# ZhengyiLuo/PHC

Measured on AMD Instinct MI355X. Metric: env-steps/sec at 4096 humanoid envs per GPU (VecEnv.step incl. resets), higher is better.
Workload: dtype f32

## Files before the change

### phc_amd/csrc/phc_im.h

```cpp
#pragma once
#include "phc_task.h"

namespace phc {

#if defined(PHC_SIM_PROFILE) && defined(__HIPCC__)
static __device__ unsigned long long g_phc_ptl[32];
static __device__ long long g_phc_ptl_env = -1;
#if defined(__HIP_DEVICE_COMPILE__)
#define PHC_PTL(i, ENV, LANE) if ((long long)(ENV) == g_phc_ptl_env) { __builtin_amdgcn_sched_barrier(0); __builtin_amdgcn_s_waitcnt(0); \
        const unsigned long long t_ = __builtin_readcyclecounter(); if ((LANE) == 0) g_phc_ptl[i] = t_; __builtin_amdgcn_sched_barrier(0); }
#else
#define PHC_PTL(i, ENV, LANE)
#endif
#else
#define PHC_PTL(i, ENV, LANE)
#endif

PHC_HD int64_t motion_id_of(const phc_im_buffers_t& buf, int64_t env) { return buf.sampled_motion_ids ? buf.sampled_motion_ids[env] : env; }

PHC_HD int phc_atomic_inc(int32_t* p) {
#if defined(__HIP_DEVICE_COMPILE__)
    return atomicAdd(p, 1);
#else
    int v;
// ... 200 lines not shown
    const Q4 hroot = obs_root_rot(prm, root.rot);
    Q4 hinv = calc_heading_quat_inv(hroot), h = calc_heading_quat(hroot);
    float* obs = buf.obs_buf + env * (int64_t)(prm.num_self_obs + prm.num_task_obs);
    if (prm.self_obs_v == 2 && buf.body_state_hist) self_obs_v2_lane(prm, buf.body_state_hist, nb, env, j, body, root, hinv, obs, true, false);
    else self_obs_lane(prm, nb, j, body, root, hinv, obs, (sim.force_sensor && prm.self_obs_v == 3) ? sim.force_sensor + env * (int64_t)(prm.num_force_sensors * 6) : nullptr, env);
    PHC_PTL(4, env, j)
    {
        float* amp = buf.amp_obs_out + env * amp_env_stride(prm, buf);
        amp_obs_from_sim_lane(prm, sim, nb, nd, env, j, root, hinv, model.ints + 4 + 3 * PHC_MAX_BODIES, amp);
    }
    PHC_PTL(5, env, j)
    BodyState r0 = ref_body_blend(q0, fr0.blend), r1 = ref_body_blend(q1, fr1.blend);
    r0.pos += c.goff; r1.pos += c.goff;
    rp = reward_partial(prm, env, nb, j, body, r0);
    if (c.cycled) {
        BodyState rr = ref_body(lib, frame_ref(lib, mid, c.t_rew), j);
        rr.pos += c.goff_rew;
        RewardPartial q = reward_partial(prm, env, nb, j, body, rr);
        rp.pos = q.pos; rp.rot = q.rot; rp.vel = q.vel; rp.angvel = q.angvel;
        if (j == 0) rp.root_dist = norm(body.pos - rr.pos);
    } else if (j == 0) {
        rp.root_dist = norm(body.pos - r0.pos);
    }
    if (prm.track_body_reward && prm.track_slot[j] < 0) rp.pos = rp.rot = rp.vel = rp.angvel = 0.f;
    if (occluded(buf, prm, env, prm.track_slot[j])) { rp.dist = 0.f; rp.fallen = 0; }
    if (prm.power_reward && j >= 1) {
        int ds = model.ints[4 + 3 * PHC_MAX_BODIES + j];
        const float* d = sim.dof_state + (env * nd + ds) * 2;
        const float* f = sim.dof_force + env * nd + ds;
        rp.power = fabsf(f[0] * d[1]);
        if (prm.dofs_per_joint != 1) rp.power += fabsf(f[1] * d[3]) + fabsf(f[2] * d[5]);
    }
    PHC_PTL(6, env, j)
    int slot = prm.track_slot[j];
    if (slot >= 0) {
        BodyState rt = r1;
        if (prm.zero_out_far && !(prm.obs_v >= 1 && prm.obs_v <= 3)) {
            BodyState rroot = (j == 0) ? r1 : ref_body(lib, fr1, 0);
            if (j != 0) rroot.pos += c.goff;
            const float dist = zero_out_far_ref(prm, slot, body, root, rroot, &rt);
            if (j == 0 && buf.point_goal) buf.point_goal[env] = dist;
        }
        occlude_ref(buf, prm, env, slot, body, &rt);
        V3 jd = v3(0.f, 0.f, 0.f), jv, rjd = jd, rjv;
        if (prm.obs_v == 2 && j >= 1) {
            ld_joint_state(sim, nd, env, model.ints[4 + 3 * PHC_MAX_BODIES + j], prm.dofs_per_joint, &jd, &jv);
            ref_joint(lib, fr1, j, &rjd, &rjv);
        }
        task_obs_lane(prm, slot, body, root, rt, hinv, h, obs + prm.num_self_obs, &jd, &rjd);
    }
    PHC_PTL(7, env, j)
    if (buf.ref_body_pos) st3(buf.ref_body_pos + (env * nb + j) * 3, r1.pos);
    if (buf.ref_body_rot) st4(buf.ref_body_rot + (env * nb + j) * 4, r1.rot);
    if (buf.ref_body_vel) st3(buf.ref_body_vel + (env * nb + j) * 3, r1.vel);
    if (want_dof)
        st_joint(buf.ref_dof_pos + env * nd + model.ints[4 + 3 * PHC_MAX_BODIES + j], prm.dofs_per_joint, ref_joint_pos_blend(lib, qj, fr1.blend));
    PHC_PTL(8, env, j)
    if (prm.num_traj_samples > 1)
        task_obs_future_lane(lib, prm, mid, c.progress + 1, c.start, c.start_off, c.goff, prm.track_slot[j], j, load_body(sim.rigid_body_state, env, nb, j),
                             load_body(sim.rigid_body_state, env, nb, 0), buf.obs_buf + env * (int64_t)(prm.num_self_obs + prm.num_task_obs) + prm.num_self_obs);
    return rp;
}

PHC_HD void im_post_finalize(const phc_motion_lib_t& lib, const phc_im_params_t& prm, const phc_im_buffers_t& buf, int nb,
                             int64_t env, const ImStepCtx& c, int64_t progress, float s_pos, float s_rot, float s_vel, float s_angvel,
                             float s_power, float s_dist, float root_dist, float prev_point_goal, int any_fallen, int n_reset_bodies) {
    float J = (float)nb, JE = (float)(nb + prm.num_ext_bodies);
    if (prm.track_body_reward) J = JE = (float)prm.num_track_bodies;
    float r_pos = expf(-prm.k_pos * (s_pos / JE));
    float r_rot = expf(-prm.k_rot * (s_rot / JE));
    float r_vel = expf(-prm.k_vel * (s_vel / J));
    float r_ang = expf(-prm.k_ang_vel * (s_angvel / J));
    float rew = prm.w_pos * r_pos + prm.w_rot * r_rot + prm.w_vel * r_vel + prm.w_ang_vel * r_ang;
    const int nraw = prm.power_reward ? 5 : 4;
    float* raw = buf.reward_raw + env * nraw;
    if (prm.zero_out_far) {
        const float pg = fminf(prev_point_goal - root_dist, 1.0f / 3.0f) * 9.0f;
        const bool far = root_dist > 0.25f;
        raw[0] = pg + (far ? 0.f : r_pos * 0.5f);
        raw[1] = far ? 0.f : r_rot * 0.5f; raw[2] = far ? 0.f : r_vel * 0.5f; raw[3] = far ? 0.f : r_ang * 0.5f;
        rew = pg + (far ? 0.f : rew * 0.5f);
    } else {
        raw[0] = r_pos; raw[1] = r_rot; raw[2] = r_vel; raw[3] = r_ang;
    }
    if (prm.power_reward) {
        float pr = -prm.power_coefficient * s_power;
        if (progress <= 3) pr = 0.f;
        rew += pr;
        raw[4] = pr;
    }
    buf.rew_buf[env] = rew;
    int fallen = any_fallen;
    if (prm.use_mean_termination) {
        float mean = s_dist / (float)n_reset_bodies;
        fallen = mean > prm.termination_distances[prm.first_reset_body] ? 1 : 0;
    }
    int64_t terminated = 0;
    if (prm.enable_early_termination) {
        if (!(progress > 1)) fallen = 0;
        if (prm.disable_collision_check) fallen = 0;
        terminated = fallen ? 1 : 0;
    }
    int64_t reset = c.pass_time ? 1 : terminated;
    if (!c.pass_time && c.cycle_cnt > 0) { reset = 0; terminated = 0; }
    if (c.recovery_cnt > 0) { reset = 0; terminated = 0; }
    buf.terminate_buf[env] = terminated;
    buf.reset_buf[env] = reset;
    if (reset && buf.reset_list) {
        const int sub = (int)((env >> 3) & (PHC_RESET_SUBLISTS - 1));
        const int i = phc_atomic_inc(buf.reset_count + (buf.reset_slot * PHC_RESET_SUBLISTS + sub) * PHC_RESET_COUNT_STRIDE);
        buf.reset_list[sub * buf.reset_sublist_cap + i] = (int32_t)env;
    }
    buf.progress_buf[env] = c.progress;
    if (buf.cycle_counter) buf.cycle_counter[env] = c.cycle_cnt;
    if (buf.recovery_counter) buf.recovery_counter[env] = c.recovery_cnt;
    if (c.cycled) {
        buf.motion_start_times[env] = c.start;
        buf.motion_start_times_offset[env] = c.start_off;
        st3(buf.global_offset + env * 3, c.goff);
    }
}

PHC_HD void im_reset_lane(const phc_model_t& model, const phc_motion_lib_t& lib, const phc_im_params_t& prm,
                          const phc_sim_state_t& sim, const phc_im_buffers_t& buf, int64_t env, int j, float t, bool clear_reset_flag,
                          int parts = 3) {
    const int nb = model.num_bodies, nd = model.num_dof;
    const int64_t mid = motion_id_of(buf, env);
    const bool p_state = (parts & 1) != 0, p_task = (parts & 2) != 0;
    if (j < nb) {
        const FrameRef fr = frame_ref(lib, mid, t);
        BodyState rs = ref_body(lib, fr, j);
        BodyState root = (j == 0) ? rs : ref_body(lib, fr, 0);
        if (p_state) {
        store_body(sim.rigid_body_state, env, nb, j, rs);
        if (sim.contact_force) st3(sim.contact_force + (env * nb + j) * 3, v3(0.f, 0.f, 0.f));
        if (j == 0) {
            float* r = sim.root_states + env * 13;
            st3(r, rs.pos); st4(r + 3, rs.rot); st3(r + 7, rs.vel); st3(r + 10, rs.angvel);
        } else {
            V3 dp, dv;
            ref_joint(lib, fr, j, &dp, &dv);
            const int ds = model.ints[4 + 3 * PHC_MAX_BODIES + j];
            float* d = sim.dof_state + (env * nd + ds) * 2;
            d[0] = dp.x; d[1] = dv.x;
            if (prm.dofs_per_joint != 1) { d[2] = dp.y; d[3] = dv.y; d[4] = dp.z; d[5] = dv.z; }
            st_joint(sim.pd_target + env * nd + ds, prm.dofs_per_joint, dp);
            if (sim.dof_force) st_joint(sim.dof_force + env * nd + ds, prm.dofs_per_joint, v3(0.f, 0.f, 0.f));
        }
        }
        const Q4 hroot = obs_root_rot(prm, root.rot);
        Q4 hinv = calc_heading_quat_inv(hroot), h = calc_heading_quat(hroot);
        float* obs = buf.obs_buf + env * (int64_t)(prm.num_self_obs + prm.num_task_obs);
        if (p_state) {
        if (prm.self_obs_v == 2 && buf.body_state_hist) self_obs_v2_lane(prm, buf.body_state_hist, nb, env, j, rs, root, hinv, obs, false, true);
        else self_obs_lane(prm, nb, j, rs, root, hinv, obs, (sim.force_sensor && prm.self_obs_v == 3) ? sim.force_sensor + env * (int64_t)(prm.num_force_sensors * 6) : nullptr, env);
        }
        if (p_task) {
        const float t1 = motion_time(1, prm.dt, t, 0.f);
        const FrameRef fr1 = frame_ref(lib, mid, t1);
        BodyState r1 = ref_body(lib, fr1, j);
        V3 goff = v3(0.f, 0.f, 0.f);
        if (buf.offset_rand && prm.zero_out_far && prm.zero_out_far_train)
            disk_offset(buf.offset_rand[env * 2], buf.offset_rand[env * 2 + 1], &goff.x, &goff.y);
        r1.pos += goff;
        int slot = prm.track_slot[j];
        if (slot >= 0) {
            BodyState rt = r1;
            if (prm.zero_out_far && !(prm.obs_v >= 1 && prm.obs_v <= 3)) {
                BodyState rroot = (j == 0) ? r1 : ref_body(lib, fr1, 0);
                if (j != 0) rroot.pos += goff;
                const float dist = zero_out_far_ref(prm, slot, rs, root, rroot, &rt);
                if (j == 0 && buf.point_goal) buf.point_goal[env] = dist;
            }
            occlude_ref(buf, prm, env, slot, rs, &rt);
            V3 jd = v3(0.f, 0.f, 0.f), jv, rjd = jd, rjv;
            if (prm.obs_v == 2 && j >= 1) { ref_joint(lib, fr, j, &jd, &jv); ref_joint(lib, fr1, j, &rjd, &rjv); }
            task_obs_lane(prm, slot, rs, root, rt, hinv, h, obs + prm.num_self_obs, &jd, &rjd);
        }
        if (buf.ref_body_pos) st3(buf.ref_body_pos + (env * nb + j) * 3, r1.pos);
        if (buf.ref_body_rot) st4(buf.ref_body_rot + (env * nb + j) * 4, r1.rot);
        if (buf.ref_body_vel) st3(buf.ref_body_vel + (env * nb + j) * 3, r1.vel);
        if (buf.ref_dof_pos && j >= 1) {
            V3 dp, dv;
            ref_joint(lib, fr1, j, &dp, &dv);
            st_joint(buf.ref_dof_pos + env * nd + model.ints[4 + 3 * PHC_MAX_BODIES + j], prm.dofs_per_joint, dp);
        }
        if (prm.num_traj_samples > 1) {
            const FrameRef frt = frame_ref(lib, mid, t);
            V3 go = v3(0.f, 0.f, 0.f);
            if (buf.offset_rand && prm.zero_out_far && prm.zero_out_far_train) disk_offset(buf.offset_rand[env * 2], buf.offset_rand[env * 2 + 1], &go.x, &go.y);
            task_obs_future_lane(lib, prm, mid, 1, t, 0.f, go, prm.track_slot[j], j, ref_body(lib, frt, j), ref_body(lib, frt, 0),
                                 buf.obs_buf + env * (int64_t)(prm.num_self_obs + prm.num_task_obs) + prm.num_self_obs);
        }
        }
    }
    if (j == 0 && p_state) {
        buf.motion_start_times[env] = t;
        buf.motion_start_times_offset[env] = 0.f;
        V3 goff = v3(0.f, 0.f, 0.f);
        const bool far_start = buf.offset_rand && prm.zero_out_far && prm.zero_out_far_train;
        if (far_start) disk_offset(buf.offset_rand[env * 2], buf.offset_rand[env * 2 + 1], &goff.x, &goff.y);
        st3(buf.global_offset + env * 3, goff);
        buf.progress_buf[env] = 0; buf.terminate_buf[env] = 0;
        if (clear_reset_flag) buf.reset_buf[env] = 0;
        if (buf.cycle_counter) buf.cycle_counter[env] = far_start ? prm.zero_out_far_steps : 0;
        if (buf.recovery_counter) buf.recovery_counter[env] = 0;
    }
}

PHC_HD void im_reset_from_state_lane(const phc_model_t& model, const phc_motion_lib_t& lib, const phc_im_params_t& prm,
                                     const phc_sim_state_t& sim, const phc_im_buffers_t& buf, int64_t env, int j, int fill_history) {
    const int nb = model.num_bodies, nd = model.num_dof;
    const int64_t mid = motion_id_of(buf, env);
    const int S = prm.num_amp_obs_steps, A = prm.num_amp_obs_per_step;
    if (j < nb) {
        BodyState body = load_body(sim.rigid_body_state, env, nb, j);
        BodyState root = load_body(sim.rigid_body_state, env, nb, 0);
        if (sim.contact_force) st3(sim.contact_force + (env * nb + j) * 3, v3(0.f, 0.f, 0.f));
        if (j >= 1) {
            const int ds = model.ints[4 + 3 * PHC_MAX_BODIES + j];
            V3 dp, dv;
            ld_joint_state(sim, nd, env, ds, prm.dofs_per_joint, &dp, &dv);
            st_joint(sim.pd_target + env * nd + ds, prm.dofs_per_joint, dp);
        }
        const V3 goff = ld3(buf.global_offset + env * 3);
        const float t1 = motion_time(1, prm.dt, buf.motion_start_times[env], buf.motion_start_times_offset[env]);
        const FrameRef fr1 = frame_ref(lib, mid, t1);
        BodyState r1 = ref_body(lib, fr1, j);
        r1.pos += goff;
        const Q4 hroot = obs_root_rot(prm, root.rot);
    Q4 hinv = calc_heading_quat_inv(hroot), h = calc_heading_quat(hroot);
        float* obs = buf.obs_buf + env * (int64_t)(prm.num_self_obs + prm.num_task_obs);
        if (prm.self_obs_v == 2 && buf.body_state_hist) self_obs_v2_lane(prm, buf.body_state_hist, nb, env, j, body, root, hinv, obs, false, true);
        else self_obs_lane(prm, nb, j, body, root, hinv, obs, (sim.force_sensor && prm.self_obs_v == 3) ? sim.force_sensor + env * (int64_t)(prm.num_force_sensors * 6) : nullptr, env);
        int slot = prm.track_slot[j];
        if (slot >= 0) {
            BodyState rt = r1;
            if (prm.zero_out_far && !(prm.obs_v >= 1 && prm.obs_v <= 3)) {
                BodyState rroot = (j == 0) ? r1 : ref_body(lib, fr1, 0);
                if (j != 0) rroot.pos += goff;
                const float dist = zero_out_far_ref(prm, slot, body, root, rroot, &rt);
                if (j == 0 && buf.point_goal) buf.point_goal[env] = dist;
            }
            occlude_ref(buf, prm, env, slot, body, &rt);
            V3 jd = v3(0.f, 0.f, 0.f), jv, rjd = jd, rjv;
            if (prm.obs_v == 2 && j >= 1) {
                ld_joint_state(sim, nd, env, model.ints[4 + 3 * PHC_MAX_BODIES + j], prm.dofs_per_joint, &jd, &jv);
                ref_joint(lib, fr1, j, &rjd, &rjv);
            }
            task_obs_lane(prm, slot, body, root, rt, hinv, h, obs + prm.num_self_obs, &jd, &rjd);
        }
        if (buf.ref_body_pos) st3(buf.ref_body_pos + (env * nb + j) * 3, r1.pos);
        if (buf.ref_body_rot) st4(buf.ref_body_rot + (env * nb + j) * 4, r1.rot);
        if (buf.ref_body_vel) st3(buf.ref_body_vel + (env * nb + j) * 3, r1.vel);
        if (buf.ref_dof_pos && j >= 1) {
            V3 dp, dv;
            ref_joint(lib, fr1, j, &dp, &dv);
            st_joint(buf.ref_dof_pos + env * nd + model.ints[4 + 3 * PHC_MAX_BODIES + j], prm.dofs_per_joint, dp);
        }
        float* amp = buf.amp_obs_out + env * amp_env_stride(prm, buf);
        const int nfill = fill_history ? S : 1;
        for (int k = 0; k < nfill; ++k)
            amp_obs_from_sim_lane(prm, sim, nb, nd, env, j, root, hinv, model.ints + 4 + 3 * PHC_MAX_BODIES, amp + k * A);
        if (prm.num_traj_samples > 1)
            task_obs_future_lane(lib, prm, mid, 1, buf.motion_start_times[env], buf.motion_start_times_offset[env], ld3(buf.global_offset + env * 3),
                                 prm.track_slot[j], j, load_body(sim.rigid_body_state, env, nb, j), load_body(sim.rigid_body_state, env, nb, 0),
                                 buf.obs_buf + env * (int64_t)(prm.num_self_obs + prm.num_task_obs) + prm.num_self_obs);
    }
    if (j == 0) {
        buf.progress_buf[env] = 0; buf.terminate_buf[env] = 0; buf.reset_buf[env] = 0;
    }
}

PHC_HD void im_reset_amp_lane(const phc_motion_lib_t& lib, const phc_im_params_t& prm, const phc_im_buffers_t& buf, int nb,
                              int64_t env, int j, float t, int k) {
    const int A = prm.num_amp_obs_per_step;
    float* amp = buf.amp_obs_out + env * amp_env_stride(prm, buf);
    amp_obs_from_ref_lane(lib, prm, nb, j, motion_id_of(buf, env), history_time(t, prm.dt, k), amp + k * A);
}
#define PHC_AMP_TABLE_BLEND_TOL 1e-4f
PHC_HD void amp_obs_from_table_lane(const phc_motion_lib_t& lib, const phc_im_params_t& prm, int nb, int j, int nl, int64_t mid, float t, float* a) {
    const int A = prm.num_amp_obs_per_step, E = prm.num_amp_obs_extra, W = A - E;
    const FrameRef fr = frame_ref(lib, mid, t);
    const float b = fr.blend;
    if (j < nb && E > 0 && prm.amp_obs_extra) obs_extra_lane(prm.amp_obs_extra + mid * E, E, j, nb, a + W);
    if (!(b <= PHC_AMP_TABLE_BLEND_TOL)) {
        amp_obs_from_frames_lane(lib, prm, nb, j, fr, a);
        return;
    }
    const float* r0 = prm.amp_ref_table + fr.f0 * (int64_t)W;
    const float* r1 = prm.amp_ref_table + fr.f1 * (int64_t)W;
    const float s0 = 1.0f - b;
    for (int c0 = j; c0 < W; c0 += 8 * nl) {
        float u[8], v[8];
        for (int i = 0; i < 8; ++i) { const int c = c0 + i * nl; if (c < W) { u[i] = r0[c]; v[i] = r1[c]; } }
        for (int i = 0; i < 8; ++i) { const int c = c0 + i * nl; if (c < W) a[c] = s0 * u[i] + b * v[i]; }
    }
}
PHC_HD void im_reset_amp_table_lane(const phc_motion_lib_t& lib, const phc_im_params_t& prm, const phc_im_buffers_t& buf, int nb,
                                    int64_t env, int j, int nl, float t, int k) {
    amp_obs_from_table_lane(lib, prm, nb, j, nl, motion_id_of(buf, env), history_time(t, prm.dt, k),
                            buf.amp_obs_out + env * amp_env_stride(prm, buf) + k * prm.num_amp_obs_per_step);
}

}
```

### phc_amd/csrc/phc_kernels.hip

```cpp
#include <hip/hip_runtime.h>
#include <stdlib.h>
#include "phc_aba.h"
#include "phc_im.h"

using namespace phc;

template <int CTRL>
__device__ __forceinline__ int dpp_i(int v) { return __builtin_amdgcn_update_dpp(0, v, CTRL, 0xf, 0xf, true); }
template <int G>
__device__ __forceinline__ float group_sum(float v) {
    v += __int_as_float(dpp_i<0xB1>(__float_as_int(v)));
    v += __int_as_float(dpp_i<0x4E>(__float_as_int(v)));
    v += __int_as_float(dpp_i<0x141>(__float_as_int(v)));
    v += __int_as_float(dpp_i<0x140>(__float_as_int(v)));
#pragma unroll
    for (int m = 16; m < G; m <<= 1) v += __shfl_xor(v, m, G);
    return v;
}
template <int G>
__device__ __forceinline__ int group_or(int v) {
    v |= dpp_i<0xB1>(v); v |= dpp_i<0x4E>(v); v |= dpp_i<0x141>(v); v |= dpp_i<0x140>(v);
#pragma unroll
    for (int m = 16; m < G; m <<= 1) v |= __shfl_xor(v, m, G);
    return v;
}

template <int DPJ>
__device__ __forceinline__ void pin_family(phc_motion_lib_t& lib, phc_im_params_t& prm) {
    lib.dofs_per_joint = DPJ; prm.dofs_per_joint = DPJ;
    if (DPJ == 3) { lib.num_ext_bodies = 0; prm.num_ext_bodies = 0; }
}

template <int DPJ, int G>
__global__ __launch_bounds__(256) void k_im_post_physics(phc_model_t model, phc_motion_lib_t lib, phc_im_params_t prm,
                                                        phc_sim_state_t sim, phc_im_buffers_t buf, int n_reset_bodies) {
    pin_family<DPJ>(lib, prm);
    const int lane = threadIdx.x & (G - 1);
    const int64_t env = ((int64_t)blockIdx.x * blockDim.x + threadIdx.x) / G;
    if (env >= sim.num_envs) return;
    PHC_PTL(0, env, lane)
    if (blockIdx.x == 0 && threadIdx.x == 0 && buf.reset_rng_counter) *buf.reset_rng_counter += 1;
    const int64_t progress = buf.progress_buf[env] + 1;
    const FrameTab tab = frame_tab(lib, motion_id_of(buf, env));
    const int jb = lane < model.num_bodies ? lane : 0;
    const BodyState body = load_body(sim.rigid_body_state, env, model.num_bodies, jb);
    const BodyState root = load_body(sim.rigid_body_state, env, model.num_bodies, 0);
    const ImStepCtx c = im_post_prologue(lib, prm, sim, buf, env, progress);
    const float prev_goal = (prm.zero_out_far && buf.point_goal) ? buf.point_goal[env] : 0.f;
    PHC_PTL(1, env, lane)
    RewardPartial rp = im_post_lane(model, lib, prm, sim, buf, env, lane, c, tab, body, root);
    PHC_PTL(9, env, lane)
    amp_shift_lane(prm, buf, env, lane, G);
    float s_pos = group_sum<G>(rp.pos), s_rot = group_sum<G>(rp.rot), s_vel = group_sum<G>(rp.vel), s_ang = group_sum<G>(rp.angvel);
    float s_pow = group_sum<G>(rp.power), s_dist = group_sum<G>(rp.dist);
    int fallen = group_or<G>(rp.fallen);
    PHC_PTL(10, env, lane)
    if (lane == 0)
        im_post_finalize(lib, prm, buf, model.num_bodies, env, c, progress, s_pos, s_rot, s_vel, s_ang, s_pow, s_dist, rp.root_dist,
                         prev_goal, fallen, n_reset_bodies);
    PHC_PTL(11, env, lane)
}
#ifdef PHC_SIM_PROFILE
extern "C" int32_t phc_debug_post_timeline(unsigned long long* out32, long long env) {
    if (out32 && hipMemcpyFromSymbol(out32, HIP_SYMBOL(phc::g_phc_ptl), sizeof(unsigned long long) * 32) != hipSuccess) return -1;
    unsigned long long z[32] = {0};
    if (hipMemcpyToSymbol(HIP_SYMBOL(phc::g_phc_ptl), z, sizeof(z)) != hipSuccess) return -1;
    return hipMemcpyToSymbol(HIP_SYMBOL(phc::g_phc_ptl_env), &env, sizeof(env)) == hipSuccess ? 0 : -1;
}
#endif

template <int DPJ, int G>
__global__ __launch_bounds__(256) void k_amp_ref_table(phc_model_t model, phc_motion_lib_t lib, phc_im_params_t prm, int64_t num_frames,
                                                       const int64_t* __restrict__ next_frame, float* __restrict__ table) {
    pin_family<DPJ>(lib, prm);
    const int lane = threadIdx.x & (G - 1);
    const int64_t f = ((int64_t)blockIdx.x * blockDim.x + threadIdx.x) / G;
    if (f >= num_frames) return;
    FrameRef fr;
    fr.f0 = f; fr.f1 = next_frame[f]; fr.idx0 = fr.idx1 = 0; fr.blend = 0.f;
    amp_obs_from_frames_lane(lib, prm, model.num_bodies, lane, fr, table + f * (int64_t)(prm.num_amp_obs_per_step - prm.num_amp_obs_extra));
}

template <int G>
__global__ __launch_bounds__(256) void k_im_reset_from_state(phc_model_t model, phc_motion_lib_t lib, phc_im_params_t prm, phc_sim_state_t sim,
                                                            phc_im_buffers_t buf, int num_reset, const int64_t* __restrict__ env_ids,
                                                            int fill_history) {
    const int lane = threadIdx.x & (G - 1);
    const int64_t r = ((int64_t)blockIdx.x * blockDim.x + threadIdx.x) / G;
    if (r >= num_reset) return;
    im_reset_from_state_lane(model, lib, prm, sim, buf, env_ids[r], lane, fill_history);
}

__device__ __forceinline__ float hash_u01(uint64_t key, uint32_t env) {
    uint32_t x = env * 0x9E3779B1u ^ (uint32_t)key;
    x ^= x >> 16; x *= 0x85EBCA6Bu; x ^= x >> 13; x *= 0xC2B2AE35u; x ^= x >> 16;
    x += (uint32_t)(key >> 32);
    x ^= x >> 15; x *= 0x2C1B3C6Du; x ^= x >> 12; x *= 0x297A2D39u; x ^= x >> 15;
    return (float)(x >> 8) * (1.0f / 16777216.0f);
}
__host__ __device__ static inline uint64_t splitmix64(uint64_t z) {
    z += 0x9E3779B97F4A7C15ull;
    z = (z ^ (z >> 30)) * 0xBF58476D1CE4E5B9ull;
    z = (z ^ (z >> 27)) * 0x94D049BB133111EBull;
    return z ^ (z >> 31);
}

#ifdef PHC_SIM_PROFILE
__device__ unsigned long long g_phc_rtl[64];
__device__ int g_phc_rtl_group = -1;
extern "C" int32_t phc_debug_reset_timeline(unsigned long long* out64, int32_t group) {
    if (out64 && hipMemcpyFromSymbol(out64, HIP_SYMBOL(g_phc_rtl), sizeof(g_phc_rtl)) != hipSuccess) return -1;
    unsigned long long z[64] = {0};
    if (hipMemcpyToSymbol(HIP_SYMBOL(g_phc_rtl), z, sizeof(z)) != hipSuccess) return -1;
    return hipMemcpyToSymbol(HIP_SYMBOL(g_phc_rtl_group), &group, sizeof(group)) == hipSuccess ? 0 : -1;
}
#define PHC_RTL(i) if (rtl_on) { __builtin_amdgcn_sched_barrier(0); __builtin_amdgcn_s_waitcnt(0); const unsigned long long t_ = __builtin_readcyclecounter(); \
        if (lane == 0) g_phc_rtl[i] = t_; __builtin_amdgcn_sched_barrier(0); }
#else
#define PHC_RTL(i)
#endif

template <int DPJ, bool RNG, int G>
__global__ __launch_bounds__(256) void k_im_reset(phc_model_t model, phc_motion_lib_t lib, phc_im_params_t prm, phc_sim_state_t sim,
                                                 phc_im_buffers_t buf, int num_reset, const int64_t* __restrict__ env_ids,
                                                 const float* __restrict__ phase, int start_at_zero, uint64_t rng_key) {
    pin_family<DPJ>(lib, prm);
    const int lane = threadIdx.x & (G - 1);
    const int64_t r = ((int64_t)blockIdx.x * blockDim.x + threadIdx.x) / G;
    const int k = (int)blockIdx.y;
#ifdef PHC_SIM_PROFILE
    const bool rtl_on = (int)(r * 16 + k) == g_phc_rtl_group;
#endif
    PHC_RTL(0)
    int64_t env;
    if (RNG && buf.reset_list) {
        const int cap = buf.reset_sublist_cap, r32 = (int)r;
        const int sub = r32 & (PHC_RESET_SUBLISTS - 1), i = r32 >> 4;
        if (r32 < PHC_RESET_SUBLISTS && k == 0 && lane == 0)
            buf.reset_count[(((buf.reset_slot + 1) % 3) * PHC_RESET_SUBLISTS + r32) * PHC_RESET_COUNT_STRIDE] = 0;
        if (i >= cap || i >= buf.reset_count[(buf.reset_slot * PHC_RESET_SUBLISTS + sub) * PHC_RESET_COUNT_STRIDE]) return;
        env = buf.reset_list[sub * cap + i];
    } else {
        if (r >= num_reset) return;
        env = env_ids ? env_ids[r] : r;
        if (!env_ids && buf.reset_buf[env] == 0) return;
    }
    PHC_RTL(1)
    const int64_t mid = motion_id_of(buf, env);
    const uint64_t key = (RNG && buf.reset_rng_counter) ? splitmix64(rng_key ^ (*buf.reset_rng_counter * 0x9E6C63D0876A9A47ull)) : rng_key;
    const float t = start_at_zero ? 0.f : sample_time_interval(lib, mid, RNG ? hash_u01(key, (uint32_t)env) : phase[r]);
    PHC_RTL(2)
    if (k < 2) im_reset_lane(model, lib, prm, sim, buf, env, lane, t, env_ids != nullptr, 1 << k);
    PHC_RTL(3)
    if (k >= 2) {
        if (prm.amp_ref_table != nullptr) im_reset_amp_table_lane(lib, prm, buf, model.num_bodies, env, lane, G, t, k - 2);
        else im_reset_amp_lane(lib, prm, buf, model.num_bodies, env, lane, t, k - 2);
    }
    PHC_RTL(4)
}

template <int G>
__global__ __launch_bounds__(256) void k_amp_obs_demo(phc_model_t model, phc_motion_lib_t lib, phc_im_params_t prm, int n,
                                                     const int64_t* __restrict__ motion_ids, const float* __restrict__ times0,
                                                     float* __restrict__ out) {
    const int lane = threadIdx.x & (G - 1);
    const int64_t i = ((int64_t)blockIdx.x * blockDim.x + threadIdx.x) / G;
    const int k = (int)blockIdx.y;
    const int S = prm.num_amp_obs_steps, A = prm.num_amp_obs_per_step;
    if (i >= n) return;
    if (prm.amp_ref_table != nullptr) amp_obs_from_table_lane(lib, prm, model.num_bodies, lane, G, motion_ids[i], history_time(times0[i], prm.dt, k), out + (i * S + k) * A);
    else amp_obs_from_ref_lane(lib, prm, model.num_bodies, lane, motion_ids[i], history_time(times0[i], prm.dt, k), out + (i * S + k) * A);
}

template <int G>
__global__ __launch_bounds__(256) void k_motion_state(phc_motion_lib_t lib, int n, const int64_t* __restrict__ ids,
                                                     const float* __restrict__ times, const float* __restrict__ offset,
                                                     float* rg_pos, float* rb_rot, float* body_vel, float* body_ang_vel,
                                                     float* dof_pos, float* dof_vel, int64_t* idx0, int64_t* idx1, float* blend,
                                                     float* rg_pos_ext, float* rb_rot_ext) {
    const int lane = threadIdx.x & (G - 1);
    const int64_t i = ((int64_t)blockIdx.x * blockDim.x + threadIdx.x) / G;
    if (i >= n) return;
    const int nb = lib.num_bodies;
    const FrameRef fr = frame_ref(lib, ids[i], times[i]);
    if (lane == 0) {
        if (idx0) idx0[i] = fr.idx0;
        if (idx1) idx1[i] = fr.idx1;
        if (blend) blend[i] = fr.blend;
    }
    if (lane >= nb) {
        const int e = lane - nb, ne = lib.num_ext_bodies;
        if (e < ne && (rg_pos_ext || rb_rot_ext)) {
            V3 p; Q4 q;
            ref_body_ext(lib, fr, e, &p, &q);
            if (offset) p += ld3(offset + i * 3);
            if (rg_pos_ext) st3(rg_pos_ext + (i * ne + e) * 3, p);
            if (rb_rot_ext) st4(rb_rot_ext + (i * ne + e) * 4, q);
        }
        return;
    }
    BodyState s = ref_body(lib, fr, lane);
    if (offset) s.pos += ld3(offset + i * 3);
    if (rg_pos) st3(rg_pos + (i * nb + lane) * 3, s.pos);
    if (rb_rot) st4(rb_rot + (i * nb + lane) * 4, s.rot);
    if (body_vel) st3(body_vel + (i * nb + lane) * 3, s.vel);
    if (body_ang_vel) st3(body_ang_vel + (i * nb + lane) * 3, s.angvel);
    if (lane >= 1 && (dof_pos || dof_vel)) {
        V3 dp, dv;
        ref_joint(lib, fr, lane, &dp, &dv);
        const int dpj = lib.dofs_per_joint == 1 ? 1 : 3;
        if (dof_pos) st_joint(dof_pos + (i * (nb - 1) + (lane - 1)) * dpj, dpj, dp);
        if (dof_vel) st_joint(dof_vel + (i * (nb - 1) + (lane - 1)) * dpj, dpj, dv);
    }
}

__global__ void k_sample_time_interval(phc_motion_lib_t lib, int n, const int64_t* __restrict__ ids,
                                       const float* __restrict__ phase, float* __restrict__ out) {
    const int i = blockIdx.x * blockDim.x + threadIdx.x;
    if (i < n) out[i] = sample_time_interval(lib, ids[i], phase[i]);
}

__global__ void k_gae(int T, int n, const float* __restrict__ fdones, const float* __restrict__ values,
                      const float* __restrict__ rewards, const float* __restrict__ next_values, float gamma, float tau,
                      float* __restrict__ advs) {
    const int i = blockIdx.x * blockDim.x + threadIdx.x;
    if (i >= n) return;
    float last = 0.f;
    for (int t = T - 1; t >= 0; --t) {
        const int64_t k = (int64_t)t * n + i;
        const float not_done = 1.0f - fdones[k];
        const float delta = rewards[k] + gamma * next_values[k] - values[k];
        last = delta + gamma * tau * not_done * last;
        advs[k] = last;
    }
}

__device__ __forceinline__ Q4 pl_quat_mul_norm(Q4 a, Q4 b) {
    Q4 q = quat_mul16(a, b);
    if (q.w < 0.f) q = q4(-q.x, -q.y, -q.z, -q.w);
    float n = fmaxf(sqrtf(q.x * q.x + q.y * q.y + q.z * q.z + q.w * q.w), 1e-9f);
    return q4(q.x / n, q.y / n, q.z / n, q.w / n);
}
__global__ void k_fk(phc_model_t model, int64_t T, const float* __restrict__ local_rot, const float* __restrict__ root_trans,
                     float* __restrict__ grot, float* __restrict__ gpos) {
    const int64_t f = (int64_t)blockIdx.x * blockDim.x + threadIdx.x;
    if (f >= T) return;
    const int nb = model.num_bodies;
    for (int j = 0; j < nb; ++j) {
        const int p = model_tab(model, 0, j);
        Q4 lq = ld4(local_rot + (f * nb + j) * 4);
        if (p < 0) {
            st4(grot + (f * nb + j) * 4, lq);
            st3(gpos + (f * nb + j) * 3, ld3(root_trans + f * 3));
        } else {
            Q4 pq = ld4(grot + (f * nb + p) * 4);
            const float* mb = model_body(model, j);
            V3 off = quat_rotate(pq, v3(mb[0], mb[1], mb[2]));
            st4(grot + (f * nb + j) * 4, pl_quat_mul_norm(pq, lq));
            st3(gpos + (f * nb + j) * 3, off + ld3(gpos + (f * nb + p) * 3));
        }
    }
}

static inline int32_t launch_status() {
    hipError_t e = hipGetLastError();
    return e == hipSuccess ? 0 : (int32_t)e;
}
static inline int env_blocks(int64_t groups, int lanes) { return (int)((groups * lanes + 255) / 256); }
static inline int group_lanes(int num_bodies, int num_ext) { return num_bodies + num_ext > 32 ? 64 : 32; }

extern "C" {

int32_t phc_abi_version(void) { return PHC_ABI_VERSION; }

int32_t phc_motion_state(const phc_motion_lib_t* lib, int32_t n, const int64_t* motion_ids, const float* motion_times,
                         const float* offset, float* rg_pos, float* rb_rot, float* body_vel, float* body_ang_vel,
                         float* dof_pos, float* dof_vel, int64_t* frame_idx0, int64_t* frame_idx1, float* blend, float* rg_pos_ext,
                         float* rb_rot_ext, void* stream) {
    if (!lib || n < 0 || lib->num_bodies + lib->num_ext_bodies > PHC_MAX_BODIES) return PHC_EINVAL;
    if (n == 0) return 0;
    if (group_lanes(lib->num_bodies, lib->num_ext_bodies) == 64)
        hipLaunchKernelGGL(k_motion_state<64>, dim3(env_blocks(n, 64)), dim3(256), 0, (hipStream_t)stream, *lib, n, motion_ids, motion_times, offset,
                           rg_pos, rb_rot, body_vel, body_ang_vel, dof_pos, dof_vel, frame_idx0, frame_idx1, blend, rg_pos_ext, rb_rot_ext);
    else
        hipLaunchKernelGGL(k_motion_state<32>, dim3(env_blocks(n, 32)), dim3(256), 0, (hipStream_t)stream, *lib, n, motion_ids, motion_times, offset,
                           rg_pos, rb_rot, body_vel, body_ang_vel, dof_pos, dof_vel, frame_idx0, frame_idx1, blend, rg_pos_ext, rb_rot_ext);
    return launch_status();
}

int32_t phc_sample_time_interval(const phc_motion_lib_t* lib, int32_t n, const int64_t* motion_ids, const float* phase,
                                 float* motion_times, void* stream) {
    if (!lib || n < 0) return PHC_EINVAL;
    if (n == 0) return 0;
    hipLaunchKernelGGL(k_sample_time_interval, dim3((n + 255) / 256), dim3(256), 0, (hipStream_t)stream, *lib, n, motion_ids, phase, motion_times);
    return launch_status();
}

static int32_t check_model(const phc_model_t* m) {
    if (!m || m->num_bodies < 1 || m->num_bodies > PHC_MAX_BODIES || !m->ints || !m->floats) return PHC_EINVAL;
    if (m->num_dof != 3 * (m->num_bodies - 1) && m->num_dof != m->num_bodies - 1) return PHC_EUNSUPPORTED;
    return 0;
}

static int32_t check_im(const phc_model_t* model, const phc_motion_lib_t* lib, const phc_im_params_t* prm) {
    int32_t rc = check_model(model);
    if (rc) return rc;
    if (!lib || !prm || lib->num_bodies != model->num_bodies) return PHC_EINVAL;
    const int dpj = model->num_dof == model->num_bodies - 1 && model->num_bodies > 2 ? 1 : 3;
    if ((lib->dofs_per_joint == 1 ? 1 : 3) != dpj || (prm->dofs_per_joint == 1 ? 1 : 3) != dpj) return PHC_EINVAL;
    if (prm->num_ext_bodies < 0 || prm->num_ext_bodies != lib->num_ext_bodies || model->num_bodies + prm->num_ext_bodies > PHC_MAX_BODIES) return PHC_EINVAL;
    if (prm->num_ext_bodies > 0 && (!prm->ext_parent || !prm->ext_offset)) return PHC_EINVAL;
    if (!prm->track_slot || !prm->reset_mask || !prm->termination_distances || !prm->key_body_ids || !prm->amp_joint_slot) return PHC_EINVAL;
    if (prm->num_key_bodies > 32) return PHC_EUNSUPPORTED;
    return 0;
}

int32_t phc_im_post_physics(const phc_model_t* model, const phc_motion_lib_t* lib, const phc_im_params_t* prm,
                            const phc_sim_state_t* sim, const phc_im_buffers_t* buf, void* stream) {
    int32_t rc = check_im(model, lib, prm);
    if (rc) return rc;
    if (!sim || !buf || buf->amp_obs_in == buf->amp_obs_out) return PHC_EINVAL;
    if (prm->cycle_motion && (!buf->cycle_counter || !buf->cycle_phase)) return PHC_EINVAL;
    if (prm->zero_out_far && (!buf->point_goal || prm->track_slot == nullptr)) return PHC_EINVAL;
    if (sim->num_envs == 0) return 0;
    const int n_reset_bodies = prm->num_reset_bodies > 0 ? prm->num_reset_bodies : 1;
    const int g = group_lanes(model->num_bodies, prm->num_ext_bodies);
    const dim3 grid(env_blocks(sim->num_envs, g));
#define PHC_POST(DPJ, G) hipLaunchKernelGGL((k_im_post_physics<DPJ, G>), grid, dim3(256), 0, (hipStream_t)stream, *model, *lib, *prm, *sim, *buf, n_reset_bodies)
    if (prm->dofs_per_joint == 1) { if (g == 64) PHC_POST(1, 64); else PHC_POST(1, 32); }
    else { if (g == 64) PHC_POST(3, 64); else PHC_POST(3, 32); }
#undef PHC_POST
    return launch_status();
}

int32_t phc_amp_ref_table(const phc_model_t* model, const phc_motion_lib_t* lib, const phc_im_params_t* prm, int64_t num_frames,
                          const int64_t* next_frame, float* table, void* stream) {
    int32_t rc = check_im(model, lib, prm);
    if (rc) return rc;
    if (!table || !next_frame || num_frames < 0 || num_frames > lib->num_frames_total) return PHC_EINVAL;
    if (num_frames == 0) return 0;
    const int g = group_lanes(model->num_bodies, prm->num_ext_bodies);
    const int64_t blocks = (num_frames * g + 255) / 256;
    if (blocks > 0x7fffffffLL) return PHC_EUNSUPPORTED;
#define PHC_TAB(DPJ, G) hipLaunchKernelGGL((k_amp_ref_table<DPJ, G>), dim3((unsigned)blocks), dim3(256), 0, (hipStream_t)stream, *model, *lib, *prm, num_frames, next_frame, table)
    if (prm->dofs_per_joint == 1) { if (g == 64) PHC_TAB(1, 64); else PHC_TAB(1, 32); }
    else { if (g == 64) PHC_TAB(3, 64); else PHC_TAB(3, 32); }
#undef PHC_TAB
    return launch_status();
}

int32_t phc_im_reset(const phc_model_t* model, const phc_motion_lib_t* lib, const phc_im_params_t* prm, const phc_sim_state_t* sim,
                     const phc_im_buffers_t* buf, int32_t num_reset, const int64_t* env_ids, const float* phase,
                     int32_t start_at_zero, void* stream) {
    int32_t rc = check_im(model, lib, prm);
    if (rc) return rc;
    if (!sim || !buf || num_reset < 0 || (!start_at_zero && !phase)) return PHC_EINVAL;
    if (num_reset == 0) return 0;
    const int g = group_lanes(model->num_bodies, prm->num_ext_bodies);
    const dim3 grid(env_blocks(num_reset, g), prm->num_amp_obs_steps + 2);
#define PHC_RESET(DPJ, G) hipLaunchKernelGGL((k_im_reset<DPJ, false, G>), grid, dim3(256), 0, (hipStream_t)stream, *model, *lib, *prm, *sim, *buf, num_reset, env_ids, phase, start_at_zero, 0ull)
    if (prm->dofs_per_joint == 1) { if (g == 64) PHC_RESET(1, 64); else PHC_RESET(1, 32); }
    else { if (g == 64) PHC_RESET(3, 64); else PHC_RESET(3, 32); }
#undef PHC_RESET
    return launch_status();
}

int32_t phc_im_reset_done(const phc_model_t* model, const phc_motion_lib_t* lib, const phc_im_params_t* prm, const phc_sim_state_t* sim,
                          const phc_im_buffers_t* buf, uint64_t seed, uint64_t counter, int32_t start_at_zero, void* stream) {
    int32_t rc = check_im(model, lib, prm);
    if (rc) return rc;
    if (!sim || !buf) return PHC_EINVAL;
    if (sim->num_envs == 0) return 0;
    if (buf->reset_list && (!buf->reset_count || buf->reset_sublist_cap * PHC_RESET_SUBLISTS < sim->num_envs)) return PHC_EINVAL;
    const int n = buf->reset_list ? buf->reset_sublist_cap * PHC_RESET_SUBLISTS : sim->num_envs;
    const uint64_t key = splitmix64(splitmix64(seed) ^ ((buf->reset_rng_counter ? 0ull : counter) * 0xD1342543DE82EF95ull));
    const int g = group_lanes(model->num_bodies, prm->num_ext_bodies);
    const dim3 grid(env_blocks(n, g), prm->num_amp_obs_steps + 2);
#define PHC_RESET(DPJ, G) hipLaunchKernelGGL((k_im_reset<DPJ, true, G>), grid, dim3(256), 0, (hipStream_t)stream, *model, *lib, *prm, *sim, *buf, n, nullptr, nullptr, start_at_zero, key)
    if (prm->dofs_per_joint == 1) { if (g == 64) PHC_RESET(1, 64); else PHC_RESET(1, 32); }
    else { if (g == 64) PHC_RESET(3, 64); else PHC_RESET(3, 32); }
#undef PHC_RESET
    return launch_status();
}

int32_t phc_im_reset_from_state(const phc_model_t* model, const phc_motion_lib_t* lib, const phc_im_params_t* prm,
                                const phc_sim_state_t* sim, const phc_im_buffers_t* buf, int32_t num_reset, const int64_t* env_ids,
                                int32_t fill_history, void* stream) {
    int32_t rc = check_im(model, lib, prm);
    if (rc) return rc;
    if (!sim || !buf || num_reset < 0 || (num_reset > 0 && !env_ids)) return PHC_EINVAL;
    if (num_reset == 0) return 0;
    if (group_lanes(model->num_bodies, prm->num_ext_bodies) == 64)
        hipLaunchKernelGGL(k_im_reset_from_state<64>, dim3(env_blocks(num_reset, 64)), dim3(256), 0, (hipStream_t)stream, *model, *lib, *prm, *sim,
                           *buf, num_reset, env_ids, fill_history);
    else
        hipLaunchKernelGGL(k_im_reset_from_state<32>, dim3(env_blocks(num_reset, 32)), dim3(256), 0, (hipStream_t)stream, *model, *lib, *prm, *sim,
                           *buf, num_reset, env_ids, fill_history);
    return launch_status();
}

int32_t phc_amp_obs_demo(const phc_model_t* model, const phc_motion_lib_t* lib, const phc_im_params_t* prm, int32_t n,
                         const int64_t* motion_ids, const float* motion_times0, float* amp_obs_demo, void* stream) {
    int32_t rc = check_im(model, lib, prm);
    if (rc) return rc;
    if (n < 0) return PHC_EINVAL;
    if (n == 0) return 0;
    if (group_lanes(model->num_bodies, prm->num_ext_bodies) == 64)
        hipLaunchKernelGGL(k_amp_obs_demo<64>, dim3(env_blocks(n, 64), prm->num_amp_obs_steps), dim3(256), 0, (hipStream_t)stream, *model, *lib,
                           *prm, n, motion_ids, motion_times0, amp_obs_demo);
    else
        hipLaunchKernelGGL(k_amp_obs_demo<32>, dim3(env_blocks(n, 32), prm->num_amp_obs_steps), dim3(256), 0, (hipStream_t)stream, *model, *lib,
                           *prm, n, motion_ids, motion_times0, amp_obs_demo);
    return launch_status();
}

int32_t phc_gae(int32_t horizon, int32_t n, const float* fdones, const float* values, const float* rewards,
                const float* next_values, float gamma, float tau, float* advs, void* stream) {
    if (horizon < 0 || n < 0) return PHC_EINVAL;
    if (horizon == 0 || n == 0) return 0;
    hipLaunchKernelGGL(k_gae, dim3((n + 255) / 256), dim3(256), 0, (hipStream_t)stream, horizon, n, fdones, values, rewards,
                       next_values, gamma, tau, advs);
    return launch_status();
}

int32_t phc_fk(const phc_model_t* model, int64_t num_frames, const float* local_rot, const float* root_trans, float* global_rot,
               float* global_pos, void* stream) {
    if (!model || model->num_bodies < 1 || model->num_bodies > PHC_MAX_BODIES || num_frames < 0) return PHC_EINVAL;
    if (num_frames == 0) return 0;
    hipLaunchKernelGGL(k_fk, dim3((unsigned)((num_frames + 255) / 256)), dim3(256), 0, (hipStream_t)stream, *model, num_frames,
                       local_rot, root_trans, global_rot, global_pos);
    return launch_status();
}

}
```

Before: 36.44 million.

## Stream AMP history rows per wave in reset kernel with grouped fallback roles

Changes the reset kernel's AMP-history fill when a reference table exists. Previously one grid row ran per history step; now a few roles give each env a full 64-lane wave that streams every history row. Frame indices are broadcast through readlane, rows are copied with float4 loads, and blend partner rows are reused when they were already loaded. Steps that need a full rebuild go to a small fixed set of fallback roles, balanced round-robin over those steps. This cuts launched work and redundant table loads, at the cost of more per-wave serial work and more complex branching.

```diff
diff --git a/phc_amd/csrc/phc_im.h b/phc_amd/csrc/phc_im.h
--- a/phc_amd/csrc/phc_im.h
+++ b/phc_amd/csrc/phc_im.h
@@ -526,5 +526,10 @@
     amp_obs_from_table_lane(lib, prm, nb, j, nl, motion_id_of(buf, env), history_time(t, prm.dt, k),
                             buf.amp_obs_out + env * amp_env_stride(prm, buf) + k * prm.num_amp_obs_per_step);
 }
-
-}
+#define PHC_AMP_PATH_ROW 0
+#define PHC_AMP_PATH_BLEND 1
+#define PHC_AMP_PATH_BUILD 2
+PHC_HD int amp_table_path(float b) { return b == 0.f ? PHC_AMP_PATH_ROW : (b <= PHC_AMP_TABLE_BLEND_TOL ? PHC_AMP_PATH_BLEND : PHC_AMP_PATH_BUILD); }
+#define PHC_RESET_FALLBACK_GROUPS 3
+
+}
diff --git a/phc_amd/csrc/phc_kernels.hip b/phc_amd/csrc/phc_kernels.hip
--- a/phc_amd/csrc/phc_kernels.hip
+++ b/phc_amd/csrc/phc_kernels.hip
@@ -120,14 +120,125 @@
 #define PHC_RTL(i)
 #endif
 
+__device__ __forceinline__ int64_t wave_read64(int64_t v, int src) {
+    const uint32_t lo = (uint32_t)__builtin_amdgcn_readlane((int)(uint32_t)v, src), hi = (uint32_t)__builtin_amdgcn_readlane((int)(v >> 32), src);
+    return (int64_t)(((uint64_t)hi << 32) | lo);
+}
+__device__ __forceinline__ float wave_readf(float v, int src) { return __int_as_float(__builtin_amdgcn_readlane(__float_as_int(v), src)); }
+__device__ __forceinline__ bool is_neg_zero(float v) { return __float_as_uint(v) == 0x80000000u; }
+__device__ __forceinline__ bool is_neg_zero(const float4& v) { return is_neg_zero(v.x) | is_neg_zero(v.y) | is_neg_zero(v.z) | is_neg_zero(v.w); }
+__device__ __forceinline__ float blend_rows(float u, float v, float s0, float b) {
+    PHC_NO_CONTRACT
+    return s0 * u + b * v;
+}
+__device__ __forceinline__ float4 blend_rows(const float4& u, const float4& v, float s0, float b) {
+    return make_float4(blend_rows(u.x, v.x, s0, b), blend_rows(u.y, v.y, s0, b), blend_rows(u.z, v.z, s0, b), blend_rows(u.w, v.w, s0, b));
+}
+template <typename T, int CH, int NI>
+__device__ __forceinline__ void amp_stream_chunk(const T* __restrict__ table, T* __restrict__ dst, int wv, int av, int nrows, int r0, int c0,
+                                                 int64_t my_f0, int64_t my_f1, float my_b) {
+    T u[CH][NI], ux[NI];
+#pragma unroll
+    for (int r = 0; r < CH; ++r) {
+        if (r0 + r >= nrows) break;
+        const T* __restrict__ s0p = table + wave_read64(my_f0, r0 + r) * wv;
+#pragma unroll
+        for (int i = 0; i < NI; ++i) if (c0 + i * 64 < wv) u[r][i] = s0p[c0 + i * 64];
+    }
+    const int64_t fx = wave_read64(my_f1, r0);
+    if (amp_table_path(wave_readf(my_b, r0)) == PHC_AMP_PATH_BLEND && fx != wave_read64(my_f0, r0)) {
+#pragma unroll
+        for (int i = 0; i < NI; ++i) if (c0 + i * 64 < wv) ux[i] = table[fx * wv + c0 + i * 64];
+    }
+#pragma unroll
+    for (int r = 0; r < CH; ++r) {
+        if (r0 + r >= nrows) break;
+        const float b = wave_readf(my_b, r0 + r), s0 = 1.0f - b;
+        const int path = amp_table_path(b);
+        if (path == PHC_AMP_PATH_BUILD) continue;
+        const int64_t f0 = wave_read64(my_f0, r0 + r), f1 = wave_read64(my_f1, r0 + r);
+        const int second = f1 == f0 ? 1 : (r > 0 && f1 == wave_read64(my_f0, r0 + (r > 0 ? r - 1 : 0))) ? 2 : r == 0 ? 3 : 4;
+#pragma unroll
+        for (int i = 0; i < NI; ++i) {
+            const int c = c0 + i * 64;
+            if (c >= wv) continue;
+            T o = u[r][i];
+            if (path == PHC_AMP_PATH_BLEND) {
+                T v;
+                if (second == 1) v = o;
+                else if (second == 2) v = u[r > 0 ? r - 1 : 0][i];
+                else if (second == 3) v = ux[i];
+                else v = table[f1 * wv + c];
+                o = blend_rows(o, v, s0, b);
+            } else if (is_neg_zero(o)) {
+                o = blend_rows(o, table[f1 * wv + c], s0, b);
+            }
+            dst[(int64_t)(r0 + r) * av + c] = o;
+        }
+    }
+}
+template <typename T, int CH, int NI>
+__device__ __forceinline__ void amp_stream_rows(const T* __restrict__ table, T* __restrict__ dst, int wv, int av, int nrows, int lane,
+                                                int64_t my_f0, int64_t my_f1, float my_b) {
+    if (nrows <= CH && wv <= NI * 64) { amp_stream_chunk<T, CH, NI>(table, dst, wv, av, nrows, 0, lane, my_f0, my_f1, my_b); return; }
+    for (int r0 = 0; r0 < nrows; r0 += CH)
+        for (int c0 = lane; c0 < wv; c0 += NI * 64) amp_stream_chunk<T, CH, NI>(table, dst, wv, av, nrows, r0, c0, my_f0, my_f1, my_b);
+}
+__device__ __forceinline__ void im_reset_amp_stream(const phc_motion_lib_t& lib, const phc_im_params_t& prm, const phc_im_buffers_t& buf,
+                                                    int64_t env, int lane, int64_t mid, float t) {
+    const int S = prm.num_amp_obs_steps, A = prm.num_amp_obs_per_step, E = prm.num_amp_obs_extra, W = A - E;
+    float* amp = buf.amp_obs_out + env * amp_env_stride(prm, buf);
+    const FrameTab tab = frame_tab(lib, mid);
+    if (E > 0 && prm.amp_obs_extra)
+        for (int k = 0; k < S; ++k) obs_extra_lane(prm.amp_obs_extra + mid * E, E, lane, 64, amp + k * A + W);
+    const bool wide = ((W | A) & 3) == 0 && (((uintptr_t)prm.amp_ref_table | (uintptr_t)amp) & 15) == 0;
+    for (int k0 = 0; k0 < S; k0 += 64) {
+        const int nrows = S - k0 < 64 ? S - k0 : 64;
+        const FrameRef fr = frame_ref(tab, history_time(t, prm.dt, k0 + (lane < nrows ? lane : nrows - 1)));
+        if (wide)
+            amp_stream_rows<float4, 10, 1>(reinterpret_cast<const float4*>(prm.amp_ref_table), reinterpret_cast<float4*>(amp + (int64_t)k0 * A),
+                                           W >> 2, A >> 2, nrows, lane, fr.f0, fr.f1, fr.blend);
+        else
+            amp_stream_rows<float, 10, 4>(prm.amp_ref_table, amp + (int64_t)k0 * A, W, A, nrows, lane, fr.f0, fr.f1, fr.blend);
+    }
+}
+template <int G>
+__device__ __forceinline__ void im_reset_amp_fallback(const phc_motion_lib_t& lib, const phc_im_params_t& prm, const phc_im_buffers_t& buf, int nb,
+                                                      int64_t env, int lane, int64_t mid, float t, int p) {
+    const int S = prm.num_amp_obs_steps, A = prm.num_amp_obs_per_step;
+    float* amp = buf.amp_obs_out + env * amp_env_stride(prm, buf);
+    const FrameTab tab = frame_tab(lib, mid);
+    int rank = 0;
+    for (int k0 = 0; k0 < S; k0 += G) {
+        const int k = k0 + lane;
+        const bool full = k < S && amp_table_path(frame_ref(tab, history_time(t, prm.dt, k < S ? k : S - 1)).blend) == PHC_AMP_PATH_BUILD;
+        unsigned long long m = __ballot(full) >> ((threadIdx.x & 63) & ~(G - 1));
+        if (G < 64) m &= (1ull << (G & 63)) - 1;
+        for (; m; m &= m - 1, ++rank) {
+            if (rank % PHC_RESET_FALLBACK_GROUPS != p) continue;
+            const int kb = k0 + __builtin_ctzll(m);
+            amp_obs_from_frames_lane(lib, prm, nb, lane, frame_ref(tab, history_time(t, prm.dt, kb)), amp + kb * A);
+        }
+    }
+}
+static inline int reset_roles(const phc_im_params_t* prm, int g) {
+    return prm->amp_ref_table ? 2 + 64 / g + PHC_RESET_FALLBACK_GROUPS : 2 + prm->num_amp_obs_steps;
+}
+
 template <int DPJ, bool RNG, int G>
 __global__ __launch_bounds__(256) void k_im_reset(phc_model_t model, phc_motion_lib_t lib, phc_im_params_t prm, phc_sim_state_t sim,
                                                  phc_im_buffers_t buf, int num_reset, const int64_t* __restrict__ env_ids,
                                                  const float* __restrict__ phase, int start_at_zero, uint64_t rng_key) {
     pin_family<DPJ>(lib, prm);
-    const int lane = threadIdx.x & (G - 1);
-    const int64_t r = ((int64_t)blockIdx.x * blockDim.x + threadIdx.x) / G;
+    int lane = threadIdx.x & (G - 1);
+    int64_t r = ((int64_t)blockIdx.x * blockDim.x + threadIdx.x) / G;
     const int k = (int)blockIdx.y;
+    constexpr int NS = 64 / G;
+    const bool stream = prm.amp_ref_table != nullptr && k >= 2 && k < 2 + NS;
+    if (stream) {
+        lane = threadIdx.x & 63;
+        r = (int64_t)blockIdx.x * (256 / G) + (k - 2) * 4 + (threadIdx.x >> 6);
+    }
 #ifdef PHC_SIM_PROFILE
     const bool rtl_on = (int)(r * 16 + k) == g_phc_rtl_group;
 #endif
@@ -153,8 +264,9 @@
     if (k < 2) im_reset_lane(model, lib, prm, sim, buf, env, lane, t, env_ids != nullptr, 1 << k);
     PHC_RTL(3)
     if (k >= 2) {
-        if (prm.amp_ref_table != nullptr) im_reset_amp_table_lane(lib, prm, buf, model.num_bodies, env, lane, G, t, k - 2);
-        else im_reset_amp_lane(lib, prm, buf, model.num_bodies, env, lane, t, k - 2);
+        if (prm.amp_ref_table == nullptr) im_reset_amp_lane(lib, prm, buf, model.num_bodies, env, lane, t, k - 2);
+        else if (stream) im_reset_amp_stream(lib, prm, buf, env, lane, mid, t);
+        else im_reset_amp_fallback<G>(lib, prm, buf, model.num_bodies, env, lane, mid, t, k - 2 - NS);
     }
     PHC_RTL(4)
 }
@@ -357,7 +469,7 @@
     if (!sim || !buf || num_reset < 0 || (!start_at_zero && !phase)) return PHC_EINVAL;
     if (num_reset == 0) return 0;
     const int g = group_lanes(model->num_bodies, prm->num_ext_bodies);
-    const dim3 grid(env_blocks(num_reset, g), prm->num_amp_obs_steps + 2);
+    const dim3 grid(env_blocks(num_reset, g), reset_roles(prm, g));
 #define PHC_RESET(DPJ, G) hipLaunchKernelGGL((k_im_reset<DPJ, false, G>), grid, dim3(256), 0, (hipStream_t)stream, *model, *lib, *prm, *sim, *buf, num_reset, env_ids, phase, start_at_zero, 0ull)
     if (prm->dofs_per_joint == 1) { if (g == 64) PHC_RESET(1, 64); else PHC_RESET(1, 32); }
     else { if (g == 64) PHC_RESET(3, 64); else PHC_RESET(3, 32); }
@@ -375,7 +487,7 @@
     const int n = buf->reset_list ? buf->reset_sublist_cap * PHC_RESET_SUBLISTS : sim->num_envs;
     const uint64_t key = splitmix64(splitmix64(seed) ^ ((buf->reset_rng_counter ? 0ull : counter) * 0xD1342543DE82EF95ull));
     const int g = group_lanes(model->num_bodies, prm->num_ext_bodies);
-    const dim3 grid(env_blocks(n, g), prm->num_amp_obs_steps + 2);
+    const dim3 grid(env_blocks(n, g), reset_roles(prm, g));
 #define PHC_RESET(DPJ, G) hipLaunchKernelGGL((k_im_reset<DPJ, true, G>), grid, dim3(256), 0, (hipStream_t)stream, *model, *lib, *prm, *sim, *buf, n, nullptr, nullptr, start_at_zero, key)
     if (prm->dofs_per_joint == 1) { if (g == 64) PHC_RESET(1, 64); else PHC_RESET(1, 32); }
     else { if (g == 64) PHC_RESET(3, 64); else PHC_RESET(3, 32); }
```

Result: slower. 35.59 million (-2.3%).
